# abowman6/CBET_RayTracing_3D

Hardware: AMD Instinct MI355X
Metric: ray-steps/sec, OMEGA 60-beam 256^3 sweep (higher is better)
Workload: dtype f64

## Files before the change

cbet_raytracing_3d_amd/api.py:

```python
import ctypes as C
import os

import numpy as np

_PKG = os.path.dirname(os.path.abspath(__file__))
LIB_PATH = os.environ.get("CBET_LIB_PATH") or os.path.join(_PKG, "lib", "libcbet_mi355x.so")
DATA_DIR = os.path.join(_PKG, "data")

OK, EINVAL, EHIP, ENOMEM, ENODEVICE, ECOMM = 0, -1, -2, -3, -4, -5
NPHASE = 2001
KERNEL_DEFAULT, KERNEL_GLOBAL_ATOMICS, KERNEL_LDS_COMBINE, KERNEL_LDS_WINDOW = 0, 1, 2, 3


class CbetError(RuntimeError):
    def __init__(self, code, msg):
        super().__init__("cbet error %d: %s" % (code, msg))
        self.code = code


class Params(C.Structure):
    _fields_ = [
        ("nx", C.c_int), ("ny", C.c_int), ("nz", C.c_int),
        ("xmin", C.c_double), ("xmax", C.c_double),
        ("ymin", C.c_double), ("ymax", C.c_double),
# ... 93 lines not shown
    ct, cp = farfield_bins(r["vx"], r["vy"], r["vz"], ntheta, nphi)

    def idx(c, n):
        c = np.where(c > 0.0, c, 0.0)
        return np.minimum(np.floor(c), n - 1).astype(np.int64)

    hist = np.zeros((ntheta, nphi))
    np.add.at(hist, (idx(ct, ntheta), idx(cp, nphi)), r["uray"])
    return hist


EXPORTS = [
    "cbet_last_error", "cbet_version", "cbet_params_default", "cbet_derive",
    "cbet_live_ray_list", "cbet_omega60_beam_norm", "cbet_host_power_table", "cbet_host_beam_trig", "cbet_read_profile",
    "cbet_safeGPUAlloc", "cbet_moveToAndFromGPU", "cbet_gpuFree",
    "cbet_context_create", "cbet_context_destroy", "cbet_context_counters", "cbet_context_tables", "cbet_context_set_launch_list",
    "cbet_launch_ray_XYZ", "cbet_tabulate_plasma", "cbet_trace_nodes", "cbet_prepare_step_records", "cbet_ray_tracing",
    "cbet_write_text", "cbet_edep_average", "cbet_edep_average_device", "cbet_node_coordinates", "cbet_write_npy",
    "cbet_debug_bounds_violations",
    "cbet_gain_params_default", "cbet_gain_constants", "cbet_trace_cbet", "cbet_gain_field",
    "cbet_cbet_workspace_bytes", "cbet_cbet_solve", "cbet_gain_field_slab", "cbet_gain_field_packed",
    "cbet_cbet_slab_workspace_bytes", "cbet_cbet_slab_workspace_bytes_parts", "cbet_pack_segments", "cbet_unpack_segments",
    "cbet_context_list_length", "cbet_cbet_workspace_gain", "cbet_trace_exits", "cbet_exit_tally", "cbet_farfield",
    "cbet_sph_modes_device", "cbet_sph_modes",
]

_lib = None


def lib():
    global _lib
# ... 9 lines not shown
    L.cbet_last_error.restype = C.c_char_p
    L.cbet_version.restype = C.c_char_p
    L.cbet_params_default.argtypes = [C.POINTER(Params), C.c_int]
    L.cbet_derive.argtypes = [C.POINTER(Params), C.POINTER(Derived)]
    L.cbet_live_ray_list.argtypes = [C.POINTER(Params), ip, C.c_long, C.POINTER(C.c_long)]
    L.cbet_omega60_beam_norm.restype = dp
    L.cbet_host_power_table.argtypes = [dp, dp]
    L.cbet_host_beam_trig.argtypes = [dp, C.c_int, dp]
    L.cbet_read_profile.argtypes = [C.c_char_p, C.c_int, dp, dp]
    L.cbet_safeGPUAlloc.argtypes = [C.POINTER(vp), C.c_size_t, C.c_int]
    L.cbet_moveToAndFromGPU.argtypes = [vp, vp, C.c_size_t, C.c_int]
    L.cbet_gpuFree.argtypes = [vp, C.c_int]
    L.cbet_context_create.argtypes = [C.POINTER(vp), C.POINTER(Params), C.c_int]
    L.cbet_context_destroy.argtypes = [vp]
    L.cbet_context_counters.argtypes = [vp, vp, C.POINTER(Counters), C.c_int]
    L.cbet_context_set_launch_list.argtypes = [vp, ip, C.c_long]
    L.cbet_context_tables.argtypes = [vp, C.POINTER(vp), C.POINTER(vp)]
    L.cbet_launch_ray_XYZ.argtypes = [C.c_int, C.c_uint, vp, vp, vp, vp, vp, vp, vp, vp,
                                      C.c_double, C.c_double, C.c_double, C.POINTER(Params), vp, vp]
    L.cbet_tabulate_plasma.argtypes = [vp, C.POINTER(Params), vp, vp, vp, vp]
    L.cbet_prepare_step_records.argtypes = [vp, C.POINTER(Params), vp, vp, C.c_double, C.c_double, C.c_double, vp]
    L.cbet_trace_nodes.argtypes = [C.c_int, C.c_uint, vp, vp, vp, vp, vp, vp, vp,
                                   C.c_double, C.c_double, C.c_double, C.POINTER(Params), vp, vp]
    L.cbet_ray_tracing.argtypes = [dp, dp, dp, dp, C.POINTER(Params), dp, ip, C.c_int, dp,
                                   C.POINTER(Counters)]
    L.cbet_debug_bounds_violations.argtypes = [C.POINTER(C.c_ulonglong), C.c_int, vp]
    L.cbet_write_text.argtypes = [dp, C.c_int, C.c_int, C.c_int, C.c_char_p]
    L.cbet_write_text.restype = C.c_longlong
    L.cbet_edep_average.argtypes = [dp, dp, C.c_int, C.c_int, C.c_int]
    L.cbet_edep_average_device.argtypes = [vp, vp, C.c_int, C.c_int, C.c_int, vp]
# ... 148 lines not shown

    def __init__(self, params, gpu=0):
        self._h = C.c_void_p()
        self.gpu = gpu
        _check(lib().cbet_context_create(C.byref(self._h), C.byref(params), gpu))

    @property
    def handle(self):
        return self._h

    def counters(self, stream=None, reset=False):
        c = Counters()
        _check(lib().cbet_context_counters(self._h, _addr(stream), C.byref(c), 1 if reset else 0))
        return c

    def set_launch_list(self, slots):
        arr = np.ascontiguousarray(slots, dtype=np.int32)
        _check(lib().cbet_context_set_launch_list(self._h, arr.ctypes.data_as(C.POINTER(C.c_int)), arr.size))

    def list_length(self):
        n = C.c_long()
        _check(lib().cbet_context_list_length(self._h, C.byref(n)))
        return n.value

    def tables(self):
        a, b = C.c_void_p(), C.c_void_p()
        _check(lib().cbet_context_tables(self._h, C.byref(a), C.byref(b)))
        return a.value, b.value

    def close(self):
# ... 224 lines not shown
```

cbet_raytracing_3d_amd/csrc/cbet_abi.cpp:

```cpp
#include <hip/hip_runtime_api.h>

#include <algorithm>
#include <cmath>
#include <cstdarg>
#include <cstdio>
#include <cstdlib>
#include <cstring>
#include <map>
#include <mutex>
#include <vector>

#include "cbet_device.h"
#include "cbet_mi355x.h"
#include "cbet_omega_beams.h"

namespace cbet {

thread_local char g_err[512] = "";

int fail(int code, const char *fmt, ...)
{
    va_list ap;
    va_start(ap, fmt);
    vsnprintf(g_err, sizeof g_err, fmt, ap);
// ... 436 lines not shown
        cbet_context_destroy(ctx);
        return fail(err == hipErrorOutOfMemory ? CBET_ENOMEM : CBET_EHIP, "%s: %s", what, hipGetErrorString(err));
    };
    if ((e = hipMalloc((void **)&ctx->ne3d, nodes * sizeof(double))) != hipSuccess) return bail(e, "hipMalloc(ne3d)");
    if ((e = hipMalloc((void **)&ctx->kap3d, nodes * sizeof(double))) != hipSuccess) return bail(e, "hipMalloc(kappa3d)");
    if ((e = hipMalloc((void **)&ctx->steprec, nodes * sizeof(StepRecord))) != hipSuccess) return bail(e, "hipMalloc(step records)");
    if ((e = hipMalloc((void **)&ctx->xlaunch, xl.size() * sizeof(double))) != hipSuccess) return bail(e, "hipMalloc(xlaunch)");
    if ((e = hipMalloc((void **)&ctx->ylaunch, yl.size() * sizeof(double))) != hipSuccess) return bail(e, "hipMalloc(ylaunch)");
    if ((e = hipMalloc((void **)&ctx->bounds, 6 * sizeof(double))) != hipSuccess) return bail(e, "hipMalloc(bounds)");
    {
        const double hb[6] = {p->xmin - (d.dx / 2.0), p->xmax + (d.dx / 2.0), p->ymin - (d.dy / 2.0),
                              p->ymax + (d.dy / 2.0), p->zmin - (d.dz / 2.0), p->zmax + (d.dz / 2.0)};
        if ((e = hipMemcpy(ctx->bounds, hb, sizeof hb, hipMemcpyHostToDevice)) != hipSuccess) return bail(e, "hipMemcpy(bounds)");
    }
    if ((e = hipMalloc((void **)&ctx->live, std::max<size_t>(1, live.size()) * sizeof(int))) != hipSuccess) return bail(e, "hipMalloc(live)");
    if ((e = hipMalloc((void **)&ctx->counters, kCntSlots * sizeof(unsigned long long))) != hipSuccess) return bail(e, "hipMalloc(counters)");
    if ((e = hipMemcpy(ctx->xlaunch, xl.data(), xl.size() * sizeof(double), hipMemcpyHostToDevice)) != hipSuccess) return bail(e, "hipMemcpy(xlaunch)");
    if ((e = hipMemcpy(ctx->ylaunch, yl.data(), yl.size() * sizeof(double), hipMemcpyHostToDevice)) != hipSuccess) return bail(e, "hipMemcpy(ylaunch)");
    if (!live.empty() &&
        (e = hipMemcpy(ctx->live, live.data(), live.size() * sizeof(int), hipMemcpyHostToDevice)) != hipSuccess)
        return bail(e, "hipMemcpy(live)");
    if ((e = hipMemset(ctx->counters, 0, kCntSlots * sizeof(unsigned long long))) != hipSuccess) return bail(e, "hipMemset(counters)");
    *out = ctx;
    return CBET_OK;
}

int cbet_context_counters(cbet_context *ctx, void *stream, cbet_counters *out, int reset)
{
    if (!ctx || !out) return fail(CBET_EINVAL, "NULL context/counters");
    DeviceGuard guard;
    CBET_HIP(hipSetDevice(ctx->gpu));
    hipStream_t s = (hipStream_t)stream;
    unsigned long long h[kCntSlots];
    CBET_HIP(hipMemcpyAsync(h, ctx->counters, sizeof h, hipMemcpyDeviceToHost, s));
    if (reset) CBET_HIP(hipMemsetAsync(ctx->counters, 0, sizeof h, s));
    CBET_HIP(hipStreamSynchronize(s));
    std::memset(out, 0, sizeof *out);
    out->ray_steps = h[kCntSteps];
    out->rays_traced = h[kCntRays];
    out->global_atomics = h[kCntGlobalAtomics];
    out->lds_evictions = h[kCntEvictions];
    out->wave_steps = h[kCntWaveSteps];
    out->wave_steps_miss = h[kCntWaveStepsMiss];
    out->wave_steps_wide = h[kCntWaveStepsWide];
    out->slabs_retired = h[kCntSlabsRetired];
    return CBET_OK;
}

int cbet_debug_bounds_violations(unsigned long long *out, int reset, void *stream)
{
    if (!out) return fail(CBET_EINVAL, "out is NULL");
    hipError_t e = audit_violations(out, reset != 0, (hipStream_t)stream);
    if (e == hipErrorNotSupported) return fail(CBET_EINVAL, "not a bounds-audit build (compile with -DCBET_DEBUG_BOUNDS)");
    if (e != hipSuccess) return fail(CBET_EHIP, "audit_violations: %s", hipGetErrorString(e));
    return CBET_OK;
}

int cbet_context_list_length(const cbet_context *ctx, long *length)
{
    if (!ctx || !length) return fail(CBET_EINVAL, "NULL context/length");
// ... 543 lines not shown
```

cbet_raytracing_3d_amd/csrc/cbet_device.h:

```cpp
#ifndef CBET_DEVICE_H_
#define CBET_DEVICE_H_

#include <hip/hip_runtime_api.h>

#include "cbet_mi355x.h"

namespace cbet {

constexpr double kC = 29979245800.0;
constexpr double kE0 = 8.85418782e-12;
constexpr double kMe = 9.10938356e-31;
constexpr double kEc = 1.60217662e-19;
constexpr double kLambda = 1.053e-4 / 3.0;
constexpr double kSigma = 0.0375;
constexpr double kIntensity = 1.0e14;
constexpr double kFocal = 0.1;
constexpr double kBeamMin = -450.0e-4;
constexpr double kBeamMax = 450.0e-4;

constexpr unsigned kEmptyTag = 0xFFFFFFFFu;
constexpr int kWave = 64;

enum CounterSlot { kCntSteps = 0, kCntRays = 1, kCntGlobalAtomics = 2, kCntEvictions = 3, kCntWaveSteps = 4,
                   kCntWaveStepsMiss = 5, kCntWaveStepsWide = 6, kCntSlabsRetired = 7, kCntSlots = 8 };

struct TabulateArgs {
    int nx, ny, nz, nprofile;
    double xmin, ymin, zmin;
    double dx, dy, dz, dt;
    double ncrit;
    const double *r, *ne, *te;
    double *ne3d, *kap3d;
};

struct StepRecord {
    double kx, ky, kz, kap;
};

struct StepTableArgs {
// ... 98 lines not shown
```

cbet_raytracing_3d_amd/csrc/cbet_trace_window.hip:

```cpp
#include <hip/hip_runtime.h>

#include <type_traits>

#if defined(__HIP_DEVICE_COMPILE__) && !defined(__gfx950__)
#error "cbet_trace_window.hip is written for gfx950 (CDNA4) only"
#endif

#include "cbet_trace_common.h"

namespace cbet {
namespace {

#define CBET_BALLOT(cond) __builtin_amdgcn_ballot_w64(cond)

template <int WX_, int WY_, int WZ_, bool PAD, bool XORSW = false>
struct Tile {
    static constexpr int WX = WX_, WY = WY_, WZ = WZ_;
    static constexpr int XM = WX - 1, YM = WY - 1, ZM = WZ - 1;
    static constexpr bool ROT = PAD && WZ == 16;
    static constexpr int YS = (PAD && !ROT) ? WZ + 1 : WZ;
    static constexpr int XS = (PAD && !ROT) ? WY * YS + 4 : WY * WZ;
    static constexpr bool XOR = ROT && XORSW;
    static __device__ __forceinline__ int zr(int tx, int ty, int tz)
    {
// ... 392 lines not shown
#endif
constexpr double kNearTol = 0.5001;
constexpr double kFarJump = 1.4998;

#define CBET_LANES(mask) __builtin_amdgcn_inverse_ballot_w64(mask)

template <int WZ, bool GENERIC, int CBET, bool STATS>
__global__ void __launch_bounds__(kWave, (CBET == 4) ? 1 : 4) k_trace_window(const TraceArgs a)
{
    using T = Tile<8, 8, WZ, true, CBET == 0>;
    using TB = Tile<4, 8, 8, false>;
    constexpr bool IDX64 = GENERIC;
    constexpr int NC = (CBET == 4) ? 4 : 1;
    constexpr bool ACC = (CBET == 0);
    constexpr bool PIPE = ACC;
    constexpr int NSLOT = T::N + TB::N;
    constexpr int NLDS = NSLOT + (NC - 1) * T::DT;
    __shared__ double s_val[NLDS];
    const int lane = threadIdx.x;

    int beam, patch;
    if (!work_item(a, blockIdx.x, beam, patch)) return;
    const Grid<!IDX64> edep{a.edep + (long)(beam - a.grid_beam0) * a.grid_stride};
    const bool absorb = GENERIC ? (a.absorption == 1) : true;

    Ray s = {};
    const int li = patch * kWave + lane;
    const int pre_raynum = li < a.nlive ? a.live[li] : -1;
    bool launched = pre_raynum >= 0;
    if (launched) launched = launch_ray(a, beam, pre_raynum, s);
    unsigned long long live = __ballot(launched);
    if (live == 0ull) return;
    const int tot_rays = __popcll(live);

    const int nx = a.nx, ny = a.ny, nz = a.nz;
    const int sYh = a.sYh, sXh = a.sXh;
    unsigned cell = launched ? (unsigned)((s.ci * ny + s.cj) * nz + s.ck) : 0u;
    double fcx = (double)s.ci, fcy = (double)s.cj, fcz = (double)s.ck;
    int tot_steps = 0;
    WaveCounters wc;

    double *const tileA = s_val, *const tileB = s_val + T::N;
    Origin oA{0, 0, 0}, oB{0, 0, 0};
    unsigned long long hbm = 0ull;
    int b_active = 0;
    {
        const int src = ((live >> 27) & 1ull) ? 27 : (__ffsll((long long)live) - 1);
        for (int z = lane; z < NLDS; z += kWave) s_val[z] = 0.0;
        oA.x = __builtin_amdgcn_readlane(s.ci, src) + 1 - T::WX / 2;
        oA.y = __builtin_amdgcn_readlane(s.cj, src) + 1 - T::WY / 2;
        oA.z = __builtin_amdgcn_readlane(s.ck, src) + 1 - 4;
        if (T::BRICK) oA.z &= ~7;
        __syncthreads();
    }
    int deep = 0;
#ifdef CBET_DIAG_CLOCKS
    unsigned long long dg_wait = 0, dg_shift = 0, dg_nshift = 0, dg_t_start;
    asm volatile("s_memtime %0\n\ts_waitcnt lgkmcnt(0)" : "=&s"(dg_t_start) : : "memory");
#endif

// ... 31 lines not shown

    bool slow = true;
    double Fx0 = 0, Fx1 = 0, Fy0 = 0, Fy1 = 0, Fz0 = 0, Fz1 = 0;
    int X0 = 0, X1 = 0, Y0 = 0, Y1 = 0, Z0 = 0, Z1 = 0;
    double inc = 0.0;
    int tile_off = 0;
    unsigned long long miss_m = 0ull;
    int own_slot = 0, own_node = 0;
    auto lds_add8 = [&](const double *w) {
        auto add = [&](int byte, double v) {
            if (CBET_AUDIT(a, (unsigned)byte < (unsigned)NSLOT * 8u))
                __hip_atomic_fetch_add(static_cast<double *>(__builtin_assume_aligned(reinterpret_cast<char *>(s_val) + byte, 8)),
                                       v, __ATOMIC_RELAXED, __HIP_MEMORY_SCOPE_WORKGROUP);
        };
        if constexpr (T::XOR) {
            int ax0, ax1, by0, by1, cz0, cz1;
            if (b_active == 0) {
                ax0 = T::xterm(X0 & T::XM); ax1 = T::xterm(X1 & T::XM);
                by0 = T::yterm(Y0 & T::YM); by1 = T::yterm(Y1 & T::YM);
                cz0 = (Z0 & T::ZM) << 3; cz1 = (Z1 & T::ZM) << 3;
            } else {
                const bool toB = tile_off != 0;
                const int xm = toB ? TB::XM : T::XM, zm = toB ? TB::ZM : T::ZM;
                const int xmul = toB ? TB::XS * 8 : T::XS * 8 + 32, ymul = toB ? TB::YS * 8 : T::YS * 8 + 16;
                const int keep = toB ? ~0 : ~0x80, off8 = tile_off * 8;
                static_assert(TB::YM == T::YM, "one y mask for both boxes");
                ax0 = (__mul24(X0 & xm, xmul) & keep) | off8; ax1 = (__mul24(X1 & xm, xmul) & keep) | off8;
                by0 = __mul24(Y0 & T::YM, ymul); by1 = __mul24(Y1 & T::YM, ymul);
                cz0 = (Z0 & zm) << 3; cz1 = (Z1 & zm) << 3;
            }
            auto at = [](int ax, int by, int cz) { return (int)__builtin_amdgcn_bitop3_b32(ax, by, cz, 0x96); };
            add(at(ax0, by0, cz0), w[0]);
            add(at(ax1, by0, cz0), w[1]);
            add(at(ax0, by0, cz1), w[2]);
            add(at(ax1, by0, cz1), w[3]);
            add(at(ax0, by1, cz0), w[4]);
            add(at(ax1, by1, cz0), w[5]);
            add(at(ax0, by1, cz1), w[6]);
            add(at(ax1, by1, cz1), w[7]);
        } else {
            auto add8 = [&](int xm, int ym, int zm, int xs, int ys, int off, int rot) {
                const int xa = X0 & xm, xb = X1 & xm, ya = Y0 & ym, yb = Y1 & ym;
                const int x0 = __mul24(xa, xs * 8) + off * 8, x1 = __mul24(xb, xs * 8) + off * 8;
                const int y0 = __mul24(ya, ys * 8), y1 = __mul24(yb, ys * 8);
                const int ra = 7 * xa * rot, rb = 7 * xb * rot, sa = 3 * ya * rot, sb = 3 * yb * rot;
// ... 30 lines not shown
        }
    };
    auto hbm_add8 = [&](const double *w) {
        const int nX0 = __mul24(X0, sXh), nX1 = __mul24(X1, sXh), nY0 = __mul24(Y0, sYh), nY1 = __mul24(Y1, sYh);
        grid_add(a, edep, nX0 + nY0 + Z0, w[0]);
        grid_add(a, edep, nX1 + nY0 + Z0, w[1]);
        grid_add(a, edep, nX0 + nY0 + Z1, w[2]);
        grid_add(a, edep, nX1 + nY0 + Z1, w[3]);
        grid_add(a, edep, nX0 + nY1 + Z0, w[4]);
        grid_add(a, edep, nX1 + nY1 + Z0, w[5]);
        grid_add(a, edep, nX0 + nY1 + Z1, w[6]);
        grid_add(a, edep, nX1 + nY1 + Z1, w[7]);
        wc.n_atomics += 8;
    };

    auto deposit_step = [&](unsigned long long lds_m, unsigned long long hbm_m) {
        const double zi0 = Fz0 * inc, zi1 = Fz1 * inc;
        const double zy00 = zi0 * Fy0, zy10 = zi1 * Fy0, zy01 = zi0 * Fy1, zy11 = zi1 * Fy1;
        double wgt[8];
        wgt[0] = zy00 * Fx0;
        wgt[1] = zy00 * Fx1;
        wgt[2] = zy10 * Fx0;
        wgt[3] = zy10 * Fx1;
        wgt[4] = zy01 * Fx0;
        wgt[5] = zy01 * Fx1;
        wgt[6] = zy11 * Fx0;
        wgt[7] = zy11 * Fx1;
        if (CBET_LANES(lds_m)) lds_add8(wgt);
        if (hbm_m != 0ull) {
            wc.pend += 8;
// ... 27 lines not shown
        const double zy00 = zi0 * Fy0, zy10 = zi1 * Fy0, zy01 = zi0 * Fy1, zy11 = zi1 * Fy1;
        const double k = CBET_LANES(restart_m) ? 0.0 : 1.0;
        auto add = [&](double &sum, double w) { asm("v_fma_f64 %0, %0, %1, %2" : "+v"(sum) : "v"(k), "v"(w)); };
        add(S[0], zy00 * Fx0);
        add(S[1], zy00 * Fx1);
        add(S[2], zy10 * Fx0);
        add(S[3], zy10 * Fx1);
        add(S[4], zy01 * Fx0);
        add(S[5], zy01 * Fx1);
        add(S[6], zy11 * Fx0);
        add(S[7], zy11 * Fx1);
    };
    auto flush_sums = [&](unsigned long long lds_m, unsigned long long hbm_m) {
        if (CBET_LANES(lds_m)) lds_add8(S);
        if (hbm_m != 0ull) {
            wc.pend += 8;
            if (CBET_LANES(hbm_m)) hbm_add8(S);
        }
    };

    auto step_tail = [&](int &tt) {
    await_record();
    if (absorb) {
        inc = rec_kzk.y * s.uray;
        s.uray -= inc;
    } else {
        inc = s.uray;
    }
    if (CBET >= 2) inc = q0;
    if constexpr (ACC && !PIPE) accumulate();
    unsigned long long died = CBET_BALLOT(s.uray <= s.ustop);
    if (slow || deep == 0) {
// ... 1 lines not shown
        died |= CBET_BALLOT(s.px < b[0]) | CBET_BALLOT(s.px > b[1]) | CBET_BALLOT(s.py < b[2]) |
                CBET_BALLOT(s.py > b[3]) | CBET_BALLOT(s.pz < b[4]) | CBET_BALLOT(s.pz > b[5]);
    }
    died &= live;
    if (died != 0ull) {
        asm volatile("");
        commit(tot_steps, tot_steps + __popcll(died) * (tt + 1));
        if constexpr (PIPE) {
            accumulate();
            asm volatile("v_mov_b64 %0, 0" : "+v"(inc));
            commit(restart_m, 0ull);
        }
        if constexpr (ACC) flush_sums(died & ~miss_m, died & miss_m);
        else deposit_step(died & ~miss_m, died & miss_m);
        commit(live, live & ~died);
        commit(hbm, hbm & live);
        commit(miss_m, miss_m & live);
        if (live == 0ull) commit(tt, a.nt - 1);
    }
    __builtin_amdgcn_wave_barrier();
    };

    for (int tt = 0; tt < a.nt; ++tt) {
        if constexpr (STATS || kDiagClocks) wc.steps_miss += 1u << 16;
        s.vx -= rec_kxy.x;
        s.vy -= rec_kxy.y;
        s.vz -= rec_kzk.x;
        s.px += s.vx * a.dt;
        s.py += s.vy * a.dt;
        s.pz += s.vz * a.dt;
        const double fx = (s.px - a.xmin) * a.inv_dx;
        const double fy = (s.py - a.ymin) * a.inv_dy;
        const double fz = (s.pz - a.zmin) * a.inv_dz;
        const double g0x = fx - fcx, g0y = fy - fcy, g0z = fz - fcz;
        const bool upx = g0x >= kNearTol, dnx = g0x < kNearTol - 1.0, upy = g0y >= kNearTol, dny = g0y < kNearTol - 1.0,
                   upz = g0z >= kNearTol, dnz = g0z < kNearTol - 1.0;
        slow = deep == 0 || (CBET_BALLOT(!(max_abs3(g0x, g0y, g0z) < kFarJump)) & live) != 0ull;
        const int di = (upx ? 1 : 0) - (dnx ? 1 : 0), dj = (upy ? 1 : 0) - (dny ? 1 : 0), dk = (upz ? 1 : 0) - (dnz ? 1 : 0);
        s.ci += di;
// ... 83 lines not shown
                u_eff = s.uray * phi;
                gained += dg;
                s.uray = s.uray + dg;
            }
            if (CBET == 2) q0 = u_eff * ds;
            if (CBET == 4) {
                q0 = u_eff * ds;
                q1 = u_eff * (s.vx * a.dt);
                q2 = u_eff * (s.vy * a.dt);
                q3 = u_eff * (s.vz * a.dt);
                const int hi = s.ci + 1, hj = s.cj + 1, hk = s.ck + 1;
                own_slot = T::slot_d(hi & T::XM, hj & T::YM, hk & T::ZM) + NSLOT;
                own_node = __mul24(hi, sXh) + __mul24(hj, sYh) + hk;
            }
        }
        const unsigned long long memA = live & ~hbm;
        unsigned long long out_core = memA & ~(CBET_BALLOT((unsigned)rx <= (unsigned)T::SX) & CBET_BALLOT((unsigned)ry <= (unsigned)T::SY) &
                                               CBET_BALLOT((unsigned)rz <= (unsigned)T::SZ));
        if (b_active != 0) {
            asm volatile("");
            if constexpr (STATS) wc.slabs_bsteps += 1u;
            const int abx = oA.x - oB.x, aby = oA.y - oB.y, abz = oA.z - oB.z;
            out_core |= hbm & ~(CBET_BALLOT((unsigned)(rx + abx) <= (unsigned)TB::SX) &
                                CBET_BALLOT((unsigned)(ry + aby) <= (unsigned)TB::SY) &
                                CBET_BALLOT((unsigned)(rz + abz) <= (unsigned)TB::SZ));
            tile_off = CBET_LANES(hbm) ? T::N : 0;
        }
        out_core |= miss_m;
        if (out_core != 0ull) {
#ifdef CBET_DIAG_CLOCKS
            unsigned long long dg_t0;
            asm volatile("s_memtime %0" : "=&s"(dg_t0) : : "memory");
#endif
            const bool alive = CBET_LANES(live);
            int lx = rx + oA.x, ly = ry + oA.y, lz = rz + oA.z;
            asm volatile("" : "+v"(lx), "+v"(ly), "+v"(lz));
            Origin nA = oA, nB = oB;
            unsigned long long n_hbm = hbm, n_miss = 0ull;
            int n_bact = b_active, n_deep, n_toff = tile_off;
            follow_box<T, NC>(a, tileA, nA, memA, lx, ly, lz, lane, edep, sXh, sYh, wc, NSLOT, a.comp_stride);
            const unsigned long long lost_mask =
                memA & ~(CBET_BALLOT((unsigned)(lx - nA.x) <= (unsigned)T::SX) & CBET_BALLOT((unsigned)(ly - nA.y) <= (unsigned)T::SY) &
                         CBET_BALLOT((unsigned)(lz - nA.z) <= (unsigned)T::SZ));
            if (lost_mask == 0ull && n_bact == 0) {
                n_deep = box_deep_inside<T>(nA, nx, ny, nz) ? 1 : 0;
            } else {
                bool homeB = CBET_LANES(hbm);
                const bool inA = alive && holds<T>(nA, lx, ly, lz);
                const bool lost = alive && !homeB && !inA;
                if (n_bact != 0) {
                    follow_box<TB, 1>(a, tileB, nB, hbm, lx, ly, lz, lane, edep, sXh, sYh, wc, 0, 0);
                } else if (lost_mask != 0ull) {
                    const int src = __ffsll((long long)lost_mask) - 1;
                    const int sx = __builtin_amdgcn_readlane(lx, src), sy = __builtin_amdgcn_readlane(ly, src),
                              sz = __builtin_amdgcn_readlane(lz, src);
                    nB.x = sx - (TB::WX / 2 - 1);
                    nB.y = sy - (TB::WY / 2 - 1);
                    nB.z = sz - TB::SZ / 2;
                    n_bact = 1;
// ... 6 lines not shown
                    __builtin_amdgcn_wave_barrier();
                    flush_box<TB, 1>(a, tileB, nB, lane, edep, sXh, sYh, wc, 0, 0);
                    n_bact = 0;
                }
                __builtin_amdgcn_wave_barrier();
                const bool useB = alive && homeB && inB;
                n_toff = useB ? T::N : 0;
                n_miss = live & ~CBET_BALLOT(useB || (alive && !homeB && inA));
                if constexpr (STATS) {
                    if (n_miss != 0ull) wc.steps_miss += 1u;
                    if (ACC && CBET_LANES(n_miss)) ++wc.n_miss;
                }
                n_deep = (n_miss == 0ull && box_deep_inside<T>(nA, nx, ny, nz) && (n_bact == 0 || box_deep_inside<TB>(nB, nx, ny, nz))) ? 1 : 0;
            }
            commit(oA.x, nA.x); commit(oA.y, nA.y); commit(oA.z, nA.z);
            commit(oB.x, nB.x); commit(oB.y, nB.y); commit(oB.z, nB.z);
            commit(hbm, n_hbm); commit(miss_m, n_miss);
            commit(b_active, n_bact); commit(deep, n_deep);
            commit_v(tile_off, n_toff);
            wc.pend = __builtin_amdgcn_readfirstlane(wc.pend);
#ifdef CBET_DIAG_CLOCKS
            {
                unsigned long long dg_t1;
                asm volatile("s_memtime %0\n\ts_waitcnt lgkmcnt(0)" : "=&s"(dg_t1) : "s"(dg_t0) : "memory");
                dg_shift += dg_t1 - dg_t0;
                dg_nshift += 1;
            }
#endif
        } else if (deep == 0) {
            const int d = (box_deep_inside<T>(oA, nx, ny, nz) && (b_active == 0 || box_deep_inside<TB>(oB, nx, ny, nz))) ? 1 : 0;
            commit(deep, d);
        }
        step_tail(tt);
    }
    tot_steps += __popcll(live) * a.nt;

    if constexpr (PIPE) accumulate();
    if constexpr (ACC) flush_sums(live & ~miss_m, live & miss_m);
    else deposit_step(live & ~miss_m, live & miss_m);
    __syncthreads();
    flush_box<T, NC>(a, tileA, oA, lane, edep, sXh, sYh, wc, NSLOT, a.comp_stride);
    if (b_active != 0) flush_box<TB, 1>(a, tileB, oB, lane, edep, sXh, sYh, wc, 0, 0);

    if (CBET && a.beam_gain) {
        double t = gained;
#pragma unroll
        for (int off = 32; off > 0; off >>= 1) t += __shfl_xor(t, off, kWave);
        if (lane == 0 && t != 0.0) atomicAdd(&a.beam_gain[beam], t);
    }
#ifdef CBET_DIAG_CLOCKS
    if (lane == 0) {
        unsigned long long dg_t_end;
        asm volatile("s_memtime %0\n\ts_waitcnt lgkmcnt(0)" : "=&s"(dg_t_end) : : "memory");
        atomicAdd(&a.counters[kCntSteps], (unsigned long long)tot_steps);
        atomicAdd(&a.counters[kCntWaveSteps], (unsigned long long)(wc.steps_miss >> 16));
        atomicAdd(&a.counters[kCntGlobalAtomics], dg_wait);
        atomicAdd(&a.counters[kCntEvictions], dg_shift);
// ... 1 lines not shown
        atomicAdd(&a.counters[kCntSlabsRetired], dg_t_end - dg_t_start);
        atomicAdd(&a.counters[kCntRays], wc.dg_ret);
        atomicAdd(&a.counters[kCntWaveStepsMiss], wc.dg_nret);
    }
    return;
#endif
    if constexpr (STATS) {
        const int tot_at = wave_sum(wc.n_atomics), tot_miss = wave_sum(wc.n_miss);
        if (lane == 0) {
            atomicAdd(&a.counters[kCntGlobalAtomics], (unsigned long long)tot_at);
            atomicAdd(&a.counters[kCntEvictions], (unsigned long long)tot_miss);
            atomicAdd(&a.counters[kCntWaveSteps], (unsigned long long)(wc.steps_miss >> 16));
            atomicAdd(&a.counters[kCntWaveStepsMiss], (unsigned long long)(wc.steps_miss & 0xFFFFu));
            atomicAdd(&a.counters[kCntWaveStepsWide], (unsigned long long)(wc.slabs_bsteps & 0xFFFFu));
            atomicAdd(&a.counters[kCntSlabsRetired], (unsigned long long)(wc.slabs_bsteps >> 16));
        }
    }
    if (lane == 0) {
        atomicAdd(&a.counters[kCntSteps], (unsigned long long)tot_steps);
        atomicAdd(&a.counters[kCntRays], (unsigned long long)tot_rays);
    }
}

}

hipError_t launch_trace_window(const TraceArgs &a, bool force_idx64, hipStream_t stream)
{
    const long waves = a.item_count;
    if (waves <= 0) return hipSuccess;
    const dim3 grid((unsigned)waves), block(kWave);
// ... 24 lines not shown
```

include/cbet_mi355x.h:

```cpp
#ifndef CBET_MI355X_H_
#define CBET_MI355X_H_

#include <stddef.h>

#ifdef __cplusplus
extern "C" {
#endif

#define CBET_OK 0
#define CBET_EINVAL (-1)
#define CBET_EHIP (-2)
#define CBET_ENOMEM (-3)
#define CBET_ENODEVICE (-4)
#define CBET_ECOMM (-5)

#define CBET_NPHASE 2001
#define CBET_MAX_CBET_BEAMS 64

#define CBET_KERNEL_DEFAULT 0
#define CBET_KERNEL_GLOBAL_ATOMICS 1
#define CBET_KERNEL_LDS_COMBINE 2
#define CBET_KERNEL_LDS_WINDOW 3

#define CBET_BEAMS_BY_GPU (-1)
// ... 60 lines not shown

int cbet_live_ray_list(const cbet_params *p, int *out, long cap, long *count);

const double *cbet_omega60_beam_norm(void);
int cbet_host_power_table(double *phase_r, double *pow_r);
int cbet_host_beam_trig(const double *beam_norm, int nbeams, double *bbeam_norm);
int cbet_read_profile(const char *path, int nprofile, double *r, double *v);

int cbet_safeGPUAlloc(void **dst, size_t size, int gpu);
int cbet_moveToAndFromGPU(void *dst, void *src, size_t size, int gpu);
int cbet_gpuFree(void *ptr, int gpu);

int cbet_context_create(cbet_context **ctx, const cbet_params *p, int gpu);
int cbet_context_destroy(cbet_context *ctx);
int cbet_context_counters(cbet_context *ctx, void *stream, cbet_counters *out, int reset);
int cbet_context_set_launch_list(cbet_context *ctx, const int *list, long n);
int cbet_context_list_length(const cbet_context *ctx, long *length);
int cbet_context_tables(cbet_context *ctx, double **ne3d, double **kappa3d);

int cbet_debug_bounds_violations(unsigned long long *out, int reset, void *stream);

int cbet_launch_ray_XYZ(int b, unsigned nindices, double *te_data_g, double *r_data_g,
                        double *ne_data_g, double *edep, double *bbeam_norm, double *beam_norm,
                        double *pow_r, double *phase_r, double xconst, double yconst,
                        double zconst, const cbet_params *p, cbet_context *ctx, void *stream);

int cbet_tabulate_plasma(cbet_context *ctx, const cbet_params *p, const double *te_data_g,
                         const double *r_data_g, const double *ne_data_g, void *stream);
int cbet_trace_nodes(int b, unsigned nindices, const double *ne3d, const double *kappa3d,
                     double *edep, const double *bbeam_norm, const double *beam_norm,
// ... 124 lines not shown
```

Baseline: 163.6 billion.

## Replace secondary LDS box B with a direct-mapped LDS line cache for missed rays

For the accumulate (CBET==0) window kernel, rays that leave the primary LDS tile box no longer get a second sliding box B. They deposit through a 32-set direct-mapped cache of 8-double z-lines held in LDS, with tags kept in lanes. On a tag miss the wave evicts the old line to global memory with atomics and installs the new tag. This removes box-B follow/flush logic and the per-step wide-box bookkeeping, at the cost of serialized eviction loops, bpermute tag lookups and possibly more global atomics when the cache thrashes. Counters for line evictions and hits and a Python replay model were added.

```diff
diff --git a/cbet_raytracing_3d_amd/api.py b/cbet_raytracing_3d_amd/api.py
--- a/cbet_raytracing_3d_amd/api.py
+++ b/cbet_raytracing_3d_amd/api.py
@@ -131,7 +131,7 @@
     "cbet_last_error", "cbet_version", "cbet_params_default", "cbet_derive",
     "cbet_live_ray_list", "cbet_omega60_beam_norm", "cbet_host_power_table", "cbet_host_beam_trig", "cbet_read_profile",
     "cbet_safeGPUAlloc", "cbet_moveToAndFromGPU", "cbet_gpuFree",
-    "cbet_context_create", "cbet_context_destroy", "cbet_context_counters", "cbet_context_tables", "cbet_context_set_launch_list",
+    "cbet_context_create", "cbet_context_destroy", "cbet_context_counters", "cbet_context_linecache_stats", "cbet_context_tables", "cbet_context_set_launch_list",
     "cbet_launch_ray_XYZ", "cbet_tabulate_plasma", "cbet_trace_nodes", "cbet_prepare_step_records", "cbet_ray_tracing",
     "cbet_write_text", "cbet_edep_average", "cbet_edep_average_device", "cbet_node_coordinates", "cbet_write_npy",
     "cbet_debug_bounds_violations",
@@ -171,6 +171,8 @@
     L.cbet_context_create.argtypes = [C.POINTER(vp), C.POINTER(Params), C.c_int]
     L.cbet_context_destroy.argtypes = [vp]
     L.cbet_context_counters.argtypes = [vp, vp, C.POINTER(Counters), C.c_int]
+    if hasattr(L, "cbet_context_linecache_stats"):
+        L.cbet_context_linecache_stats.argtypes = [vp, vp, C.POINTER(C.c_ulonglong), C.c_int]
     L.cbet_context_set_launch_list.argtypes = [vp, ip, C.c_long]
     L.cbet_context_tables.argtypes = [vp, C.POINTER(vp), C.POINTER(vp)]
     L.cbet_launch_ray_XYZ.argtypes = [C.c_int, C.c_uint, vp, vp, vp, vp, vp, vp, vp, vp,
@@ -349,6 +351,11 @@
         _check(lib().cbet_context_counters(self._h, _addr(stream), C.byref(c), 1 if reset else 0))
         return c
 
+    def linecache_stats(self, stream=None, reset=False):
+        out = (C.c_ulonglong * 2)()
+        _check(lib().cbet_context_linecache_stats(self._h, _addr(stream), out, 1 if reset else 0))
+        return int(out[0]), int(out[1])
+
     def set_launch_list(self, slots):
         arr = np.ascontiguousarray(slots, dtype=np.int32)
         _check(lib().cbet_context_set_launch_list(self._h, arr.ctypes.data_as(C.POINTER(C.c_int)), arr.size))
diff --git a/cbet_raytracing_3d_amd/csrc/cbet_abi.cpp b/cbet_raytracing_3d_amd/csrc/cbet_abi.cpp
--- a/cbet_raytracing_3d_amd/csrc/cbet_abi.cpp
+++ b/cbet_raytracing_3d_amd/csrc/cbet_abi.cpp
@@ -474,13 +474,13 @@
         if ((e = hipMemcpy(ctx->bounds, hb, sizeof hb, hipMemcpyHostToDevice)) != hipSuccess) return bail(e, "hipMemcpy(bounds)");
     }
     if ((e = hipMalloc((void **)&ctx->live, std::max<size_t>(1, live.size()) * sizeof(int))) != hipSuccess) return bail(e, "hipMalloc(live)");
-    if ((e = hipMalloc((void **)&ctx->counters, kCntSlots * sizeof(unsigned long long))) != hipSuccess) return bail(e, "hipMalloc(counters)");
+    if ((e = hipMalloc((void **)&ctx->counters, kCntDeviceSlots * sizeof(unsigned long long))) != hipSuccess) return bail(e, "hipMalloc(counters)");
     if ((e = hipMemcpy(ctx->xlaunch, xl.data(), xl.size() * sizeof(double), hipMemcpyHostToDevice)) != hipSuccess) return bail(e, "hipMemcpy(xlaunch)");
     if ((e = hipMemcpy(ctx->ylaunch, yl.data(), yl.size() * sizeof(double), hipMemcpyHostToDevice)) != hipSuccess) return bail(e, "hipMemcpy(ylaunch)");
     if (!live.empty() &&
         (e = hipMemcpy(ctx->live, live.data(), live.size() * sizeof(int), hipMemcpyHostToDevice)) != hipSuccess)
         return bail(e, "hipMemcpy(live)");
-    if ((e = hipMemset(ctx->counters, 0, kCntSlots * sizeof(unsigned long long))) != hipSuccess) return bail(e, "hipMemset(counters)");
+    if ((e = hipMemset(ctx->counters, 0, kCntDeviceSlots * sizeof(unsigned long long))) != hipSuccess) return bail(e, "hipMemset(counters)");
     *out = ctx;
     return CBET_OK;
 }
@@ -504,6 +504,22 @@
     out->wave_steps_miss = h[kCntWaveStepsMiss];
     out->wave_steps_wide = h[kCntWaveStepsWide];
     out->slabs_retired = h[kCntSlabsRetired];
+    return CBET_OK;
+}
+
+int cbet_context_linecache_stats(cbet_context *ctx, void *stream, unsigned long long out[2], int reset)
+{
+    if (!ctx || !out) return fail(CBET_EINVAL, "NULL context/out");
+    DeviceGuard guard;
+    CBET_HIP(hipSetDevice(ctx->gpu));
+    hipStream_t s = (hipStream_t)stream;
+    unsigned long long h[2];
+    static_assert(kCntLineHits == kCntLineEvictions + 1, "the two slots are read together");
+    CBET_HIP(hipMemcpyAsync(h, ctx->counters + kCntLineEvictions, sizeof h, hipMemcpyDeviceToHost, s));
+    if (reset) CBET_HIP(hipMemsetAsync(ctx->counters + kCntLineEvictions, 0, sizeof h, s));
+    CBET_HIP(hipStreamSynchronize(s));
+    out[0] = h[0];
+    out[1] = h[1];
     return CBET_OK;
 }
 
diff --git a/cbet_raytracing_3d_amd/csrc/cbet_device.h b/cbet_raytracing_3d_amd/csrc/cbet_device.h
--- a/cbet_raytracing_3d_amd/csrc/cbet_device.h
+++ b/cbet_raytracing_3d_amd/csrc/cbet_device.h
@@ -22,7 +22,8 @@
 constexpr int kWave = 64;
 
 enum CounterSlot { kCntSteps = 0, kCntRays = 1, kCntGlobalAtomics = 2, kCntEvictions = 3, kCntWaveSteps = 4,
-                   kCntWaveStepsMiss = 5, kCntWaveStepsWide = 6, kCntSlabsRetired = 7, kCntSlots = 8 };
+                   kCntWaveStepsMiss = 5, kCntWaveStepsWide = 6, kCntSlabsRetired = 7, kCntSlots = 8,
+                   kCntLineEvictions = 8, kCntLineHits = 9, kCntDeviceSlots = 10 };
 
 struct TabulateArgs {
     int nx, ny, nz, nprofile;
diff --git a/cbet_raytracing_3d_amd/csrc/cbet_trace_window.hip b/cbet_raytracing_3d_amd/csrc/cbet_trace_window.hip
--- a/cbet_raytracing_3d_amd/csrc/cbet_trace_window.hip
+++ b/cbet_raytracing_3d_amd/csrc/cbet_trace_window.hip
@@ -430,6 +430,9 @@
     constexpr int NC = (CBET == 4) ? 4 : 1;
     constexpr bool ACC = (CBET == 0);
     constexpr bool PIPE = ACC;
+    constexpr bool LC = (CBET == 0);
+    constexpr int LC_SETS = TB::N / 8;
+    static_assert(LC_SETS == 32, "set index and tag lanes are written for 32 lines");
     constexpr int NSLOT = T::N + TB::N;
     constexpr int NLDS = NSLOT + (NC - 1) * T::DT;
     __shared__ double s_val[NLDS];
@@ -460,6 +463,10 @@
     Origin oA{0, 0, 0}, oB{0, 0, 0};
     unsigned long long hbm = 0ull;
     int b_active = 0;
+    int lc_tag = -1;
+    int lc_any = 0;
+    int lc_evict = 0, lc_hits = 0;
+    bool lc_missed = false;
     {
         const int src = ((live >> 27) & 1ull) ? 27 : (__ffsll((long long)live) - 1);
         for (int z = lane; z < NLDS; z += kWave) s_val[z] = 0.0;
@@ -521,21 +528,9 @@
                                        v, __ATOMIC_RELAXED, __HIP_MEMORY_SCOPE_WORKGROUP);
         };
         if constexpr (T::XOR) {
-            int ax0, ax1, by0, by1, cz0, cz1;
-            if (b_active == 0) {
-                ax0 = T::xterm(X0 & T::XM); ax1 = T::xterm(X1 & T::XM);
-                by0 = T::yterm(Y0 & T::YM); by1 = T::yterm(Y1 & T::YM);
-                cz0 = (Z0 & T::ZM) << 3; cz1 = (Z1 & T::ZM) << 3;
-            } else {
-                const bool toB = tile_off != 0;
-                const int xm = toB ? TB::XM : T::XM, zm = toB ? TB::ZM : T::ZM;
-                const int xmul = toB ? TB::XS * 8 : T::XS * 8 + 32, ymul = toB ? TB::YS * 8 : T::YS * 8 + 16;
-                const int keep = toB ? ~0 : ~0x80, off8 = tile_off * 8;
-                static_assert(TB::YM == T::YM, "one y mask for both boxes");
-                ax0 = (__mul24(X0 & xm, xmul) & keep) | off8; ax1 = (__mul24(X1 & xm, xmul) & keep) | off8;
-                by0 = __mul24(Y0 & T::YM, ymul); by1 = __mul24(Y1 & T::YM, ymul);
-                cz0 = (Z0 & zm) << 3; cz1 = (Z1 & zm) << 3;
-            }
+            const int ax0 = T::xterm(X0 & T::XM), ax1 = T::xterm(X1 & T::XM);
+            const int by0 = T::yterm(Y0 & T::YM), by1 = T::yterm(Y1 & T::YM);
+            const int cz0 = (Z0 & T::ZM) << 3, cz1 = (Z1 & T::ZM) << 3;
             auto at = [](int ax, int by, int cz) { return (int)__builtin_amdgcn_bitop3_b32(ax, by, cz, 0x96); };
             add(at(ax0, by0, cz0), w[0]);
             add(at(ax1, by0, cz0), w[1]);
@@ -596,6 +591,67 @@
         wc.n_atomics += 8;
     };
 
+    auto lc_add8 = [&](unsigned long long fm, const double *w) {
+        const bool act = CBET_LANES(fm);
+        const int nX0 = __mul24(X0, sXh), nX1 = __mul24(X1, sXh), nY0 = __mul24(Y0, sYh), nY1 = __mul24(Y1, sYh);
+        bool missed_l = false;
+        auto lds_add = [&](int byte, double v) {
+            if (CBET_AUDIT(a, (unsigned)(byte - T::N * 8) < (unsigned)TB::N * 8u))
+                __hip_atomic_fetch_add(static_cast<double *>(__builtin_assume_aligned(reinterpret_cast<char *>(s_val) + byte, 8)),
+                                       v, __ATOMIC_RELAXED, __HIP_MEMORY_SCOPE_WORKGROUP);
+        };
+        auto one = [&](int x, int y, int z, int nX, int nY, double v) {
+            const int line = nX + nY + (z & ~7);
+            const int set = ((x & 3) << 3) | ((y & 3) << 1) | ((z >> 3) & 1);
+            const int byte = T::N * 8 + (set << 6) + ((z & 7) << 3);
+            const int t = __builtin_amdgcn_ds_bpermute(set << 2, lc_tag);
+            const bool hit = act && t == line;
+            unsigned long long um = fm & ~CBET_BALLOT(hit);
+            if (hit) {
+                lds_add(byte, v);
+                if constexpr (STATS) ++lc_hits;
+            } else if constexpr (STATS) {
+                missed_l = missed_l || act;
+            }
+            while (um != 0ull) {
+                const int ld = __ffsll((long long)um) - 1;
+                const int s_ = __builtin_amdgcn_readlane(set, ld), ln = __builtin_amdgcn_readlane(line, ld);
+                const int old = __builtin_amdgcn_readlane(lc_tag, s_);
+                __builtin_amdgcn_wave_barrier();
+                const int eslot = T::N + s_ * 8 + lane;
+                double ev = 0.0;
+                if (lane < 8 && CBET_AUDIT(a, (unsigned)eslot < (unsigned)NSLOT)) ev = s_val[eslot];
+                const bool nzv = ev != 0.0;
+                const bool sent = CBET_BALLOT(nzv) != 0ull;
+                wc.pend += sent ? 1 : 0;
+                if (nzv) {
+                    s_val[eslot] = 0.0;
+                    ++wc.n_atomics;
+                    grid_add(a, edep, old + lane, ev);
+                }
+                __builtin_amdgcn_wave_barrier();
+                lc_tag = lane == s_ ? ln : lc_tag;
+                if constexpr (STATS) {
+                    lc_evict += sent ? 1 : 0;
+                    lc_any = 1;
+                    lc_missed = true;
+                }
+                const bool now = CBET_LANES(um) && line == ln;
+                if (now) lds_add(byte, v);
+                um &= ~CBET_BALLOT(now);
+            }
+        };
+        one(X0, Y0, Z0, nX0, nY0, w[0]);
+        one(X1, Y0, Z0, nX1, nY0, w[1]);
+        one(X0, Y0, Z1, nX0, nY0, w[2]);
+        one(X1, Y0, Z1, nX1, nY0, w[3]);
+        one(X0, Y1, Z0, nX0, nY1, w[4]);
+        one(X1, Y1, Z0, nX1, nY1, w[5]);
+        one(X0, Y1, Z1, nX0, nY1, w[6]);
+        one(X1, Y1, Z1, nX1, nY1, w[7]);
+        if (STATS && missed_l) ++wc.n_miss;
+    };
+
     auto deposit_step = [&](unsigned long long lds_m, unsigned long long hbm_m) {
         const double zi0 = Fz0 * inc, zi1 = Fz1 * inc;
         const double zy00 = zi0 * Fy0, zy10 = zi1 * Fy0, zy01 = zi0 * Fy1, zy11 = zi1 * Fy1;
@@ -653,8 +709,12 @@
     auto flush_sums = [&](unsigned long long lds_m, unsigned long long hbm_m) {
         if (CBET_LANES(lds_m)) lds_add8(S);
         if (hbm_m != 0ull) {
-            wc.pend += 8;
-            if (CBET_LANES(hbm_m)) hbm_add8(S);
+            if constexpr (LC) {
+                lc_add8(hbm_m, S);
+            } else {
+                wc.pend += 8;
+                if (CBET_LANES(hbm_m)) hbm_add8(S);
+            }
         }
     };
 
@@ -686,7 +746,7 @@
         if constexpr (ACC) flush_sums(died & ~miss_m, died & miss_m);
         else deposit_step(died & ~miss_m, died & miss_m);
         commit(live, live & ~died);
-        commit(hbm, hbm & live);
+        if constexpr (!LC) commit(hbm, hbm & live);
         commit(miss_m, miss_m & live);
         if (live == 0ull) commit(tt, a.nt - 1);
     }
@@ -695,6 +755,11 @@
 
     for (int tt = 0; tt < a.nt; ++tt) {
         if constexpr (STATS || kDiagClocks) wc.steps_miss += 1u << 16;
+        if constexpr (LC && STATS) {
+            wc.slabs_bsteps += lc_any ? 1u : 0u;
+            wc.steps_miss += lc_missed ? 1u : 0u;
+            lc_missed = false;
+        }
         s.vx -= rec_kxy.x;
         s.vy -= rec_kxy.y;
         s.vz -= rec_kzk.x;
@@ -808,10 +873,11 @@
                 own_node = __mul24(hi, sXh) + __mul24(hj, sYh) + hk;
             }
         }
-        const unsigned long long memA = live & ~hbm;
-        unsigned long long out_core = memA & ~(CBET_BALLOT((unsigned)rx <= (unsigned)T::SX) & CBET_BALLOT((unsigned)ry <= (unsigned)T::SY) &
-                                               CBET_BALLOT((unsigned)rz <= (unsigned)T::SZ));
-        if (b_active != 0) {
+        const unsigned long long memA = LC ? (live & ~miss_m) : (live & ~hbm);
+        const unsigned long long in_core = CBET_BALLOT((unsigned)rx <= (unsigned)T::SX) & CBET_BALLOT((unsigned)ry <= (unsigned)T::SY) &
+                                           CBET_BALLOT((unsigned)rz <= (unsigned)T::SZ);
+        unsigned long long out_core = LC ? (live & ~(miss_m ^ in_core)) : (memA & ~in_core);
+        if (!LC && b_active != 0) {
             asm volatile("");
             if constexpr (STATS) wc.slabs_bsteps += 1u;
             const int abx = oA.x - oB.x, aby = oA.y - oB.y, abz = oA.z - oB.z;
@@ -820,7 +886,7 @@
                                 CBET_BALLOT((unsigned)(rz + abz) <= (unsigned)TB::SZ));
             tile_off = CBET_LANES(hbm) ? T::N : 0;
         }
-        out_core |= miss_m;
+        if constexpr (!LC) out_core |= miss_m;
         if (out_core != 0ull) {
 #ifdef CBET_DIAG_CLOCKS
             unsigned long long dg_t0;
@@ -832,11 +898,14 @@
             Origin nA = oA, nB = oB;
             unsigned long long n_hbm = hbm, n_miss = 0ull;
             int n_bact = b_active, n_deep, n_toff = tile_off;
-            follow_box<T, NC>(a, tileA, nA, memA, lx, ly, lz, lane, edep, sXh, sYh, wc, NSLOT, a.comp_stride);
-            const unsigned long long lost_mask =
-                memA & ~(CBET_BALLOT((unsigned)(lx - nA.x) <= (unsigned)T::SX) & CBET_BALLOT((unsigned)(ly - nA.y) <= (unsigned)T::SY) &
-                         CBET_BALLOT((unsigned)(lz - nA.z) <= (unsigned)T::SZ));
-            if (lost_mask == 0ull && n_bact == 0) {
+            follow_box<T, NC>(a, tileA, nA, (LC && memA == 0ull) ? live : memA, lx, ly, lz, lane, edep, sXh, sYh, wc, NSLOT, a.comp_stride);
+            const unsigned long long held_mask = CBET_BALLOT((unsigned)(lx - nA.x) <= (unsigned)T::SX) & CBET_BALLOT((unsigned)(ly - nA.y) <= (unsigned)T::SY) &
+                                                 CBET_BALLOT((unsigned)(lz - nA.z) <= (unsigned)T::SZ);
+            const unsigned long long lost_mask = memA & ~held_mask;
+            if constexpr (LC) {
+                n_miss = live & ~held_mask;
+                n_deep = box_deep_inside<T>(nA, nx, ny, nz) ? 1 : 0;
+            } else if (lost_mask == 0ull && n_bact == 0) {
                 n_deep = box_deep_inside<T>(nA, nx, ny, nz) ? 1 : 0;
             } else {
                 bool homeB = CBET_LANES(hbm);
@@ -873,10 +942,13 @@
                 n_deep = (n_miss == 0ull && box_deep_inside<T>(nA, nx, ny, nz) && (n_bact == 0 || box_deep_inside<TB>(nB, nx, ny, nz))) ? 1 : 0;
             }
             commit(oA.x, nA.x); commit(oA.y, nA.y); commit(oA.z, nA.z);
-            commit(oB.x, nB.x); commit(oB.y, nB.y); commit(oB.z, nB.z);
-            commit(hbm, n_hbm); commit(miss_m, n_miss);
-            commit(b_active, n_bact); commit(deep, n_deep);
-            commit_v(tile_off, n_toff);
+            if constexpr (!LC) {
+                commit(oB.x, nB.x); commit(oB.y, nB.y); commit(oB.z, nB.z);
+                commit(hbm, n_hbm);
+                commit(b_active, n_bact);
+                commit_v(tile_off, n_toff);
+            }
+            commit(miss_m, n_miss); commit(deep, n_deep);
             wc.pend = __builtin_amdgcn_readfirstlane(wc.pend);
 #ifdef CBET_DIAG_CLOCKS
             {
@@ -887,8 +959,16 @@
             }
 #endif
         } else if (deep == 0) {
-            const int d = (box_deep_inside<T>(oA, nx, ny, nz) && (b_active == 0 || box_deep_inside<TB>(oB, nx, ny, nz))) ? 1 : 0;
+            const int d = (box_deep_inside<T>(oA, nx, ny, nz) && (LC || b_active == 0 || box_deep_inside<TB>(oB, nx, ny, nz))) ? 1 : 0;
             commit(deep, d);
+        }
+        if constexpr (LC) {
+            if (miss_m != 0ull && deep != 0) {
+                const int lo = kRelocateDeep + 1;
+                const unsigned long long okd = CBET_BALLOT(s.ci >= lo && s.ci <= nx - 4) & CBET_BALLOT(s.cj >= lo && s.cj <= ny - 4) &
+                                               CBET_BALLOT(s.ck >= lo && s.ck <= nz - 4);
+                if ((miss_m & ~okd) != 0ull) commit(deep, 0);
+            }
         }
         step_tail(tt);
     }
@@ -899,7 +979,25 @@
     else deposit_step(live & ~miss_m, live & miss_m);
     __syncthreads();
     flush_box<T, NC>(a, tileA, oA, lane, edep, sXh, sYh, wc, NSLOT, a.comp_stride);
-    if (b_active != 0) flush_box<TB, 1>(a, tileB, oB, lane, edep, sXh, sYh, wc, 0, 0);
+    if (!LC && b_active != 0) flush_box<TB, 1>(a, tileB, oB, lane, edep, sXh, sYh, wc, 0, 0);
+    if constexpr (LC) {
+#pragma unroll
+        for (int q = 0; q < LC_SETS / 8; ++q) {
+            const int e = q * kWave + lane;
+            const int t = __builtin_amdgcn_ds_bpermute((e >> 3) << 2, lc_tag);
+            const double v = CBET_AUDIT(a, (unsigned)(T::N + e) < (unsigned)NSLOT) ? tileB[e] : 0.0;
+            if constexpr (STATS) {
+                unsigned long long b = CBET_BALLOT(v != 0.0);
+                b |= b >> 4; b |= b >> 2; b |= b >> 1;
+                lc_evict += __popcll(b & 0x0101010101010101ull);
+            }
+            wc.pend += (CBET_BALLOT(v != 0.0) != 0ull) ? 1 : 0;
+            if (v != 0.0) {
+                ++wc.n_atomics;
+                grid_add(a, edep, t + (lane & 7), v);
+            }
+        }
+    }
 
     if (CBET && a.beam_gain) {
         double t = gained;
@@ -931,6 +1029,13 @@
             atomicAdd(&a.counters[kCntWaveStepsMiss], (unsigned long long)(wc.steps_miss & 0xFFFFu));
             atomicAdd(&a.counters[kCntWaveStepsWide], (unsigned long long)(wc.slabs_bsteps & 0xFFFFu));
             atomicAdd(&a.counters[kCntSlabsRetired], (unsigned long long)(wc.slabs_bsteps >> 16));
+        }
+        if constexpr (LC) {
+            const int tot_hits = wave_sum(lc_hits);
+            if (lane == 0) {
+                atomicAdd(&a.counters[kCntLineEvictions], (unsigned long long)lc_evict);
+                atomicAdd(&a.counters[kCntLineHits], (unsigned long long)tot_hits);
+            }
         }
     }
     if (lane == 0) {
diff --git a/cbet_raytracing_3d_amd/linecache_model.py b/cbet_raytracing_3d_amd/linecache_model.py
--- /dev/null
+++ b/cbet_raytracing_3d_amd/linecache_model.py
@@ -0,0 +1,285 @@
+import numpy as np
+
+AX, AY, AZ = 8, 8, 16
+BX, BY, BZ = 4, 8, 8
+
+
+def follow_plane_axis(r, S):
+    if r.size == 0:
+        return 0
+    edge = (r <= 0) | (r >= S)
+    if not edge.any():
+        return 0
+    at_hi = bool((r >= S).any())
+    at_lo = bool((r[edge] < S).any())
+    if at_hi == at_lo:
+        return 0
+    if at_hi:
+        if (r <= 1).any():
+            return 1 if (r > S).any() else 0
+        return 2 if (S >= 6 and not (r <= 2).any()) else 1
+    if (r >= S - 1).any():
+        return -1 if (r < 0).any() else 0
+    return -2 if (S >= 6 and not (r >= S - 2).any()) else -1
+
+
+def follow_brick_axis(r):
+    if r.size == 0 or not ((r < 0) | (r > 14)).any():
+        return 0
+    below, above = bool((r < 0).any()), bool((r > 14).any())
+    needs_lo, needs_hi = bool((r <= 7).any()), bool((r >= 7).any())
+    return -1 if (below and not needs_hi) else (1 if (above and not needs_lo) else 0)
+
+
+def set_index(kind, x, y, zb, nsets):
+    if kind == "xyz":
+        if nsets == 32:
+            return (x & 3) << 3 | (y & 3) << 1 | (zb & 1)
+        return (x & 3) << 2 | (y & 1) << 1 | (zb & 1) if nsets == 16 else (x & 7) << 3 | (y & 3) << 1 | (zb & 1)
+    if kind == "xy":
+        return ((x & 3) << 3 | (y & 7)) % nsets
+    if kind == "skew":
+        return (((x ^ (y >> 2)) & 3) << 3 | ((y ^ (x >> 2)) & 3) << 1 | (zb & 1)) % nsets
+    raise ValueError(kind)
+
+
+class LineCache:
+
+    def __init__(self, nsets=32, ways=1, kind="xyz"):
+        self.nsets, self.ways, self.kind = nsets, ways, kind
+        self.sets = [[] for _ in range(nsets)]
+        self.hits = self.evictions = self.fills = self.drained = 0
+
+    def touch(self, x, y, zb):
+        s = self.sets[set_index(self.kind, x, y, zb, self.nsets)]
+        tag = (x, y, zb)
+        if tag in s:
+            self.hits += 1
+            if self.ways > 1:
+                s.remove(tag)
+                s.append(tag)
+            return
+        self.fills += 1
+        if len(s) == self.ways:
+            s.pop(0)
+            self.evictions += 1
+        s.append(tag)
+
+    def drain(self):
+        n = sum(len(s) for s in self.sets)
+        self.drained += n
+        self.sets = [[] for _ in range(self.nsets)]
+        return n
+
+    @property
+    def requests(self):
+        return self.evictions + self.drained
+
+
+def lane_lines(c):
+    x, y, z = int(c[0]), int(c[1]), int(c[2])
+    zbs = (z >> 3,) if (z & 7) != 7 else (z >> 3, (z >> 3) + 1)
+    return [(xx, yy, zb) for xx in (x, x + 1) for yy in (y, y + 1) for zb in zbs]
+
+
+class _Box:
+
+    def __init__(self, w):
+        self.w = np.array(w)
+        self.o = np.zeros(3, dtype=np.int64)
+        self.t = np.zeros(w, dtype=bool)
+
+    def add(self, c):
+        for dx in (0, 1):
+            for dy in (0, 1):
+                for dz in (0, 1):
+                    self.t[(c[0] + dx) % self.w[0], (c[1] + dy) % self.w[1], (c[2] + dz) % self.w[2]] = True
+
+    def holds(self, l):
+        r = l - self.o
+        return ((r >= 0) & (r <= self.w - 2)).all(axis=-1)
+
+    def retire(self, axis, coords):
+        req = 0
+        lanes = 0
+        for c in coords:
+            idx = [slice(None)] * 3
+            idx[axis] = c % self.w[axis]
+            plane = self.t[tuple(idx)]
+            nz = np.argwhere(plane)
+            if nz.size:
+                lanes += len(nz)
+                oth = [a for a in range(3) if a != axis]
+                if axis == 2:
+                    req += len(nz)
+                else:
+                    zabs = self.o[2] + ((nz[:, 1] - self.o[2]) % self.w[2])
+                    req += len(set(zip(nz[:, 0].tolist(), (zabs >> 3).tolist())))
+                del oth
+            plane[...] = False
+        return req, lanes
+
+    def retire_brick(self, zb):
+        k = (np.arange(8) + zb) % self.w[2]
+        sub = self.t[:, :, k]
+        req = int(sub.any(axis=2).sum())
+        lanes = int(sub.sum())
+        self.t[:, :, k] = False
+        return req, lanes
+
+    def flush(self):
+        req = lanes = 0
+        for x in range(self.w[0]):
+            r, l = self.retire(0, [self.o[0] + x])
+            req += r
+            lanes += l
+        return req, lanes
+
+
+class Tally:
+    def __init__(self):
+        self.ray_steps = self.wave_steps = 0
+        self.reqA = self.lanesA = 0
+        self.reqB = self.lanesB = 0
+        self.miss_ray_steps = self.miss_flushes = 0
+        self.miss_wave_steps = self.wide_wave_steps = 0
+        self.lookups = 0
+
+    def add(self, o):
+        for k, v in o.__dict__.items():
+            setattr(self, k, getattr(self, k) + v)
+
+
+def _follow(box, mm_l, brick):
+    req = lanes = 0
+    S = box.w - 2
+    for ax in (0, 1):
+        d = follow_plane_axis(mm_l[:, ax] - box.o[ax], int(S[ax]))
+        if d:
+            first = box.o[ax] + box.w[ax] - 1 if d < 0 else box.o[ax]
+            r, l = box.retire(ax, [first + q * (-1 if d < 0 else 1) for q in range(abs(d))])
+            req += r
+            lanes += l
+            box.o[ax] += d
+    if brick:
+        d = 8 * follow_brick_axis(mm_l[:, 2] - box.o[2])
+        if d:
+            r, l = box.retire_brick(box.o[2] + 8 if d < 0 else box.o[2])
+            req += r
+            lanes += l
+            box.o[2] += d
+    else:
+        d = follow_plane_axis(mm_l[:, 2] - box.o[2], int(S[2]))
+        if d:
+            first = box.o[2] + box.w[2] - 1 if d < 0 else box.o[2]
+            r, l = box.retire(2, [first + q * (-1 if d < 0 else 1) for q in range(abs(d))])
+            req += r
+            lanes += l
+            box.o[2] += d
+    return req, lanes
+
+
+def replay_bundle(paths, scheme, cache=None, src_lane=27):
+    t = Tally()
+    lanes = [i for i, p in enumerate(paths) if p is not None and len(p)]
+    if not lanes:
+        return t
+    nlane = len(paths)
+    length = np.zeros(nlane, dtype=np.int64)
+    for i in lanes:
+        length[i] = len(paths[i])
+    T = int(length.max())
+    cells = np.zeros((T, nlane, 3), dtype=np.int64)
+    for i in lanes:
+        cells[:length[i], i] = paths[i]
+    A, B = _Box((AX, AY, AZ)), _Box((BX, BY, BZ))
+    src = src_lane if (src_lane < nlane and length[src_lane] > 0) else lanes[0]
+    A.o[:] = cells[0, src] - 3
+    A.o[2] = (cells[0, src, 2] - 3) & ~7
+    HOME_A, HOME_B, HOME_M = 0, 1, 2
+    home = np.zeros(nlane, dtype=np.int64)
+    homeB = np.zeros(nlane, dtype=bool)
+    b_active = False
+
+    def flush(i, c):
+        if home[i] == HOME_A:
+            A.add(c)
+        elif home[i] == HOME_B:
+            B.add(c)
+        elif scheme == "boxb":
+            t.miss_flushes += 1
+        else:
+            t.miss_flushes += 1
+            for ln in lane_lines(c):
+                cache.touch(*ln)
+            t.lookups += 8
+
+    for s in range(T):
+        live = length > s
+        t.wave_steps += 1
+        t.ray_steps += int(live.sum())
+        if s > 0:
+            moved = live & (cells[s] != cells[s - 1]).any(axis=1)
+            for i in np.flatnonzero(moved):
+                flush(i, cells[s - 1, i])
+        l = cells[s]
+        memA = live & ~homeB
+        if b_active or (scheme == "cache" and homeB.any()):
+            t.wide_wave_steps += 1
+        calm = A.holds(l[memA]).all()
+        if scheme == "boxb":
+            calm = calm and (not b_active or B.holds(l[live & homeB]).all()) and not (home[live] == HOME_M).any()
+        else:
+            calm = calm and not (live & homeB & A.holds(l)).any()
+        if not calm:
+            r, la = _follow(A, l[memA], True)
+            t.reqA += r
+            t.lanesA += la
+            inA = live & A.holds(l)
+            if scheme == "cache":
+                homeB = live & ~inA & (homeB | memA)
+                homeB |= live & ~inA
+                home[live] = np.where(homeB[live], HOME_M, HOME_A)
+                n_miss = int(homeB.sum())
+            else:
+                lost = live & ~homeB & ~inA
+                if b_active:
+                    r, la = _follow(B, l[live & homeB], False)
+                    t.reqB += r
+                    t.lanesB += la
+                elif lost.any():
+                    f = int(np.flatnonzero(lost)[0])
+                    B.o[:] = l[f] - np.array([BX // 2 - 1, BY // 2 - 1, (BZ - 2) // 2])
+                    b_active = True
+                inB = live & B.holds(l) if b_active else np.zeros(nlane, dtype=bool)
+                homeB = (homeB & live) | (lost & inB)
+                homeB &= ~(homeB & ~inB & inA)
+                if b_active and not homeB.any():
+                    r, la = B.flush()
+                    t.reqB += r
+                    t.lanesB += la
+                    b_active = False
+                useB = homeB & inB
+                okA = live & ~homeB & inA
+                home[live] = np.where(useB[live], HOME_B, np.where(okA[live], HOME_A, HOME_M))
+                n_miss = int((live & ~useB & ~okA).sum())
+            if n_miss:
+                t.miss_wave_steps += 1
+                t.miss_ray_steps += n_miss
+        else:
+            if scheme == "cache" and homeB.any():
+                t.miss_wave_steps += 1
+                t.miss_ray_steps += int((live & homeB).sum())
+        for i in np.flatnonzero(length == s + 1):
+            flush(i, cells[s, i])
+        homeB &= length > s + 1
+    r, la = A.flush()
+    t.reqA += r
+    t.lanesA += la
+    if b_active:
+        r, la = B.flush()
+        t.reqB += r
+        t.lanesB += la
+    if cache is not None:
+        cache.drain()
+    return t
diff --git a/include/cbet_mi355x.h b/include/cbet_mi355x.h
--- a/include/cbet_mi355x.h
+++ b/include/cbet_mi355x.h
@@ -98,6 +98,7 @@
 int cbet_context_create(cbet_context **ctx, const cbet_params *p, int gpu);
 int cbet_context_destroy(cbet_context *ctx);
 int cbet_context_counters(cbet_context *ctx, void *stream, cbet_counters *out, int reset);
+int cbet_context_linecache_stats(cbet_context *ctx, void *stream, unsigned long long out[2], int reset);
 int cbet_context_set_launch_list(cbet_context *ctx, const int *list, long n);
 int cbet_context_list_length(const cbet_context *ctx, long *length);
 int cbet_context_tables(cbet_context *ctx, double **ne3d, double **kappa3d);
```

New measurement: 120.0 billion. 26.7% lower.
